# michaelklachko/NoisyNet

Hardware: NVIDIA H100
Metric: NoisyNet CIFAR-10 4-bit training images/sec (higher is better)
Workload: dtype bf16

## Files before the change

### noisynet_b200/csrc/nn_conv_umma.cu

```cuda
#include <cuda_bf16.h>
#include <stdio.h>
#include <stdlib.h>

#include "nn_common.cuh"
#include "nn_wgmma.cuh"
#include "nn_conv_tma.h"

namespace {

constexpr int UM_BLOCK_M = 128;
constexpr int UM_BLOCK_K = 64;
constexpr int UM_THREADS = 384;
constexpr int UM_ACC_CH = 4;
constexpr int UM_A_STAGE = UM_BLOCK_M * 128;
constexpr int UM_MAX_NT = 120;

struct UmmaP {
    int B, H, W, Cp;
    int KH, KW, stride, pad, OH, OW;
    int M, Cout, n_t, n_mma, num_kb, stages, acc_cols;
    int main_col, sig_col, wsum_col;
    int ring_bytes;
    const __nv_bfloat16* xp;
    const __nv_bfloat16* wp;
// ... 328 lines not shown
            s_plain = nn_warp_sum(s_plain); s_abs = nn_warp_sum(s_abs); s_max = nn_warp_max(s_max);
            if (lane == 0) {
                atomicAdd(p.stats + 0, s_plain);
                atomicAdd(p.stats + 1, s_abs);
                nn_atomic_max_float(p.stats + 2, s_max);
            }
        }
    }
    if (dbg && tid == 128) { dbg[4] = clock64(); unsigned smid; asm volatile("mov.u32 %0, %%smid;" : "=r"(smid)); dbg[7] = smid; }
}


struct SplitEpiP {
    const float* partial; int splits, n_tiles, n_mma, n_t, main_col, sig_col, m_pad, M, Cout;
    float y_scale, s_scale, current; const float* scale_dev; nn_rng rng; float *y, *y_noisy; int noisy;
    double* stat_partial; unsigned* stat_counters; BnFinP fin; float* zero_out;
};
__global__ void __launch_bounds__(256)
k_splitk_epilogue(const SplitEpiP p) {
    const int ngrp = (p.Cout + 3) >> 2;
    const int total = p.M * ngrp;
    float coef = 0.f;
    NnRng rs = {0, 0, 0, 0};
    if (p.noisy) { coef = nn_noise_coef(*p.scale_dev, p.current); rs = nn_rng_load(p.rng); }
    for (int i = blockIdx.x * blockDim.x + threadIdx.x; i < total; i += gridDim.x * blockDim.x) {
        const int m = i % p.M, g = i / p.M;
        const int n0 = g * 4;
        const int tile = n0 / p.n_t, c0 = n0 - tile * p.n_t;
        float am[4] = {0.f, 0.f, 0.f, 0.f}, as[4] = {0.f, 0.f, 0.f, 0.f};
        for (int z = 0; z < p.splits; ++z) {
            const float* src = p.partial + (((size_t)z * p.n_tiles + tile) * p.n_mma) * p.m_pad + m;
#pragma unroll
            for (int j = 0; j < 4; ++j) {
                am[j] += src[(size_t)(p.main_col + c0 + j) * p.m_pad];
                if (p.noisy) as[j] += src[(size_t)(p.sig_col + c0 + j) * p.m_pad];
            }
        }
        float zz[4] = {0.f, 0.f, 0.f, 0.f};
        if (p.noisy) nn_normal4(rs, (uint64_t)m * ngrp + (uint64_t)g, zz);
        float* o = (p.noisy ? p.y_noisy : p.y) + (size_t)m * p.Cout + n0;
        float ov[4] = {0.f, 0.f, 0.f, 0.f};
#pragma unroll
        for (int j = 0; j < 4; ++j) {
            if (n0 + j < p.Cout) {
                const float yv = am[j] * p.y_scale;
                ov[j] = p.noisy ? __fadd_rn(yv, __fmul_rn(zz[j], nn_sigma(coef, as[j] * p.s_scale))) : yv;
                o[j] = ov[j];
                if (p.noisy && p.y) p.y[(size_t)m * p.Cout + n0 + j] = yv;
            }
        }
        if (p.stat_partial) {
            __shared__ double sh[8][8];
            const int lane = threadIdx.x & 31, wi = threadIdx.x >> 5;
#pragma unroll
            for (int j = 0; j < 4; ++j) {
                double s1 = (double)ov[j], s2 = (double)ov[j] * (double)ov[j];
#pragma unroll
                for (int o2 = 16; o2 > 0; o2 >>= 1) { s1 += __shfl_xor_sync(0xffffffffu, s1, o2); s2 += __shfl_xor_sync(0xffffffffu, s2, o2); }
                if (lane == 0) { sh[wi][2 * j] = s1; sh[wi][2 * j + 1] = s2; }
            }
            __syncthreads();
            if (threadIdx.x < 4 && n0 + (int)threadIdx.x < p.Cout) {
                const int j = threadIdx.x, c = n0 + j, slices = p.M >> 8, slice = (m >> 8);
                double a1 = 0.0, a2 = 0.0;
#pragma unroll
                for (int w = 0; w < 8; ++w) { a1 += sh[w][2 * j]; a2 += sh[w][2 * j + 1]; }
                double* part = p.stat_partial + (size_t)c * slices * 2;
                part[slice * 2] = a1; part[slice * 2 + 1] = a2;
                __threadfence();
                if (atomicAdd(p.stat_counters + c, 1u) == (unsigned)slices - 1u) {
                    p.stat_counters[c] = 0u;
                    __threadfence();
                    bn_finalize_channel(part, slices, 2, c, p.fin);
                    if (c == 0 && p.zero_out) *p.zero_out = 0.f;
                }
            }
        }
    }
}

constexpr int SH_MAX_PAIRS = 64;
constexpr int SH_STAGES = 2;
constexpr int SH_MAX_N = 256;
constexpr int SH_POOL_IT = 5;

struct ShiftP {
    int H, W, OH, OW, KH, KW, Cout;
    int n_mma, main_col, sig_col, n_pairs;
    int a_pixels, a_stage, b_bytes, n_tiles;
    long long total_pixels;
    const __nv_bfloat16 *xp, *wp;
    float y_scale, s_scale;
    float *y, *y_noisy;
    float* pooled;
    uint8_t* pool_arg;
    int blk, tiles_x, tiles_per_img, sbo_units;
    double* stat_partial;
    unsigned* stat_ticket;
    BnFinP fin;
    float* zero_out;
    const float* z_inject;
    float current;
    const float* scale_dev;
    nn_rng rng;
    int* err_flag;
    long long* dbg;
};

__device__ __forceinline__ long long shift_tile_v0(const ShiftP& p, int t, int& b, int& r0, int& c0) {
    if (!p.blk) { b = 0; r0 = 0; c0 = 0; return (long long)t * UM_BLOCK_M; }
    b = t / p.tiles_per_img;
    const int rem = t - b * p.tiles_per_img, rb = rem / p.tiles_x;
    r0 = rb * 16; c0 = (rem - rb * p.tiles_x) * 8;
    return ((long long)b * p.H + r0) * p.W + c0;
}
__device__ __forceinline__ bool shift_tile_live(const ShiftP& p, int t) {
    if (p.blk) {
        const int rem = t % p.tiles_per_img, rb = rem / p.tiles_x;
        return rb * 16 < p.OH && (rem - rb * p.tiles_x) * 8 < p.OW;
    }
    const unsigned v0 = (unsigned)t * UM_BLOCK_M, total = (unsigned)p.total_pixels;
    unsigned v1 = v0 + UM_BLOCK_M - 1;
    if (v1 >= total) v1 = total - 1;
    const unsigned hw = (unsigned)(p.H * p.W);
    const unsigned b0 = v0 / hw, b1 = v1 / hw;
    if (b0 != b1) return true;
    return (int)((v0 - b0 * hw) / (unsigned)p.W) < p.OH;
}

template <int MODE, int SH_EPI_WARPS, bool POOL>
__global__ void __launch_bounds__((1 + SH_EPI_WARPS) * 32, 1)
k_conv_shift(const ShiftP p) {
    constexpr bool NOISY = MODE != 0;
    constexpr int SH_THREADS = (1 + SH_EPI_WARPS) * 32;
    static_assert(SH_EPI_WARPS >= 8 && SH_EPI_WARPS % 4 == 0, "the first 8 epilogue warps are the MMA warpgroups");
    extern __shared__ uint8_t smem_raw[];
    const uint32_t base = (smem_u32(smem_raw) + 127u) & ~127u;
    const uint32_t b_base = base;
    const uint32_t a_base = b_base + (uint32_t)p.b_bytes;
    const uint32_t bar_base = a_base + (uint32_t)SH_STAGES * (uint32_t)p.a_stage;
    const uint32_t a_full = bar_base, a_empty = bar_base + 8u * SH_STAGES;
    const uint32_t b_full = bar_base + 16u * SH_STAGES;
    const uint32_t abort_slot = b_full + 8u, tab_slot = abort_slot + 4u;
    const uint32_t pool_slot = (tab_slot + 4u * SH_MAX_PAIRS + 15u) & ~15u;
    const uint32_t acc_slot = pool_slot + 12u * 1024u;
    uint8_t* gen0 = smem_raw + (base - smem_u32(smem_raw));
    const AccTile acc_tile = {reinterpret_cast<float*>(gen0 + (acc_slot - base)), p.n_mma + 4};
    volatile uint32_t* abort_g = reinterpret_cast<volatile uint32_t*>(gen0 + (abort_slot - base));
    uint32_t* tap_tab = reinterpret_cast<uint32_t*>(gen0 + (tab_slot - base));

    const int tid = threadIdx.x, lane = tid & 31;
    const int warp = __shfl_sync(0xffffffffu, tid >> 5, 0);
    if (tid < p.n_pairs) {
        const int khw = p.KH * p.KW, t0 = 2 * tid, t1 = 2 * tid + 1;
        const int sh0 = (t0 / p.KW) * p.W + (t0 % p.KW);
        const int sh1 = t1 < khw ? (t1 / p.KW) * p.W + (t1 % p.KW) : sh0 + 1;
        tap_tab[tid] = (uint32_t)sh0 | ((uint32_t)(sh1 - sh0) << 16);
    }
    if (tid == 0) {
        for (int s = 0; s < SH_STAGES; ++s) { mbar_init(a_full + 8 * s, 1); mbar_init(a_empty + 8 * s, 2); }
        mbar_init(b_full, 1);
        *abort_g = 0;
        fence_mbar_init();
    }
    {
        uint4* az = reinterpret_cast<uint4*>(gen0 + (a_base - base));
        const int n16 = SH_STAGES * p.a_stage / 16;
        for (int i = tid; i < n16; i += SH_THREADS) az[i] = make_uint4(0, 0, 0, 0);
        fence_proxy_async();
    }
    __syncthreads();
    const int hw = p.H * p.W;

    if (warp == SH_EPI_WARPS) {
        if (elect_one_sync()) {
            mbar_arrive_expect_tx(b_full, (uint32_t)p.b_bytes);
            bulk_g2s(b_base, p.wp, (uint32_t)p.b_bytes, b_full);
        }
        __syncwarp();
        int s = 0;
        uint32_t ph = 1u;
        for (int t = blockIdx.x; t < p.n_tiles; t += gridDim.x) {
            if (!shift_tile_live(p, t)) continue;
            if (!mbar_wait(a_empty + 8 * s, ph)) { *abort_g = 1; break; }
            if (*abort_g) break;
            int tb, tr0, tc0;
            const long long v0 = shift_tile_v0(p, t, tb, tr0, tc0);
            long long px = p.total_pixels - v0;
            if (px > p.a_pixels) px = p.a_pixels;
            const uint32_t bytes = (uint32_t)px * 16u;
            if (elect_one_sync()) {
                mbar_arrive_expect_tx(a_full + 8 * s, bytes);
                bulk_g2s(a_base + (uint32_t)s * p.a_stage, p.xp + v0 * 8, bytes, a_full + 8 * s);
            }
            __syncwarp();
            if (++s == SH_STAGES) { s = 0; ph ^= 1u; }
        }
    } else {
        const bool mma_wg = warp < 8;
        const int wg = warp >> 2;
        if (mma_wg && !mbar_wait(b_full, 0)) *abort_g = 2;
        int s = 0;
        uint32_t ph = 0u;
        const uint64_t bd0 = gmma_desc_none(b_base, (uint32_t)p.n_mma, 8u);
        const uint64_t ad_t = gmma_desc_none(0u, 0u, (uint32_t)p.sbo_units);
        const int q = warp & 3, jq = warp >> 2;
        constexpr int per_q = SH_EPI_WARPS / 4;
        const int ohw = p.OH * p.OW;
        const int ngrp = (p.Cout + 3) >> 2;
        float coef = 0.f;
        NnRng rs = {0, 0, 0, 0};
        if (NOISY) coef = nn_noise_coef(*p.scale_dev, p.current);
        if (MODE == 1) rs = nn_rng_load(p.rng);
        const float y_scale = p.y_scale, s_scale = p.s_scale;
        float st1[SH_POOL_IT], st2[SH_POOL_IT];
#pragma unroll
        for (int it = 0; it < SH_POOL_IT; ++it) { st1[it] = 0.f; st2[it] = 0.f; }
        int i = 0;
        for (int t = blockIdx.x; t < p.n_tiles; t += gridDim.x) {
            if (!shift_tile_live(p, t)) continue;
            if (mma_wg && !*abort_g) {
                if (!mbar_wait(a_full + 8 * s, ph)) {
                    *abort_g = 4;
                } else {
                    if (p.dbg && i < 32 && warp == 0 && lane == 0) p.dbg[((size_t)blockIdx.x * 32 + i) * 4 + 0] = clock64();
                    const uint32_t a_s = a_base + (uint32_t)s * p.a_stage + (uint32_t)wg * 128u * (uint32_t)p.sbo_units;
                    for (int c = 0; 64 * c < p.n_mma; ++c) {
                        const int n = min(64, p.n_mma - 64 * c);
                        float acc[1][32];
                        wg_fence();
#pragma unroll 1
                        for (int j = 0; j < p.n_pairs; ++j) {
                            const uint32_t e = tap_tab[j];
                            const uint64_t ad = ad_t | (uint64_t)(((a_s >> 4) + (e & 0xFFFFu)) & 0x3FFFu) | ((uint64_t)((e >> 16) & 0x3FFFu) << 16);
                            wgmma_n<0, 0>(acc[0], ad, bd0 + (uint64_t)(2 * j * p.n_mma + 64 * c), n, j != 0);
                        }
                        wg_commit();
                        wg_wait_all();
                        wg_fence_regs<32>(acc[0]);
                        wg_acc_store(acc, acc_tile, 64 * wg, 64 * c, n);
                    }
                    __syncwarp();
                    if ((warp & 3) == 0 && elect_one_sync()) mbar_arrive(a_empty + 8 * s);
                    __syncwarp();
                    if (p.dbg && i < 32 && warp == 0 && lane == 0) p.dbg[((size_t)blockIdx.x * 32 + i) * 4 + 1] = clock64();
                }
                if (++s == SH_STAGES) { s = 0; ph ^= 1u; }
            }
            named_bar_sync(1, SH_EPI_WARPS * 32);
            if (*abort_g) break;
            if (p.dbg && i < 32 && warp == 0 && lane == 0) p.dbg[((size_t)blockIdx.x * 32 + i) * 4 + 2] = clock64();
            int b, ih, iw;
            bool row_ok;
            if (p.blk) {
                int r0, c0;
                shift_tile_v0(p, t, b, r0, c0);
                ih = r0 + q * 4 + (lane >> 3); iw = c0 + (lane & 7);
                row_ok = ih < p.OH && iw < p.OW;
            } else {
                const unsigned v = (unsigned)t * UM_BLOCK_M + q * 32 + lane;
                b = (int)(v / (unsigned)hw);
                const int rem = (int)(v - (unsigned)b * (unsigned)hw);
                ih = (int)((unsigned)rem / (unsigned)p.W); iw = rem - ih * p.W;
                row_ok = v < (unsigned)p.total_pixels && ih < p.OH && iw < p.OW;
            }
            const int pix = ih * p.OW + iw;
            const uint64_t grp_row = (uint64_t)((long long)b * ohw + pix) * ngrp;
            const size_t out_row = (size_t)b * p.Cout * ohw + pix;
            float* const out_main = (NOISY ? p.y_noisy : p.y) + out_row;
            float* const out_y = (NOISY && p.y) ? p.y + out_row : nullptr;
            const uint32_t t_lane = (uint32_t)(q * 32) << 16;
            if (POOL) {
                const int PW = p.OW >> 1, PHW = (p.OH >> 1) * PW;
                const int w = (lane & 1) | ((lane >> 2) & 2);
                const bool w1 = (w & 1) != 0, w2 = (w & 2) != 0;
                const size_t pbase = (size_t)b * p.Cout * PHW + (size_t)(ih >> 1) * PW + (iw >> 1);
                const bool warp_live = __any_sync(0xffffffffu, row_ok);
                const int n_fix = ngrp / per_q, g_extra = n_fix * per_q;
                auto pool_group = [&](const float (&v)[4], int nb, float& s1, float& s2) {
                    const float s01 = w1 ? v[1] : v[0], s10 = w1 ? v[0] : v[1], s23 = w1 ? v[3] : v[2], s32 = w1 ? v[2] : v[3];
                    const float own = w2 ? s23 : s01;
                    const float c1 = w2 ? s32 : s10;
                    const float c2 = w2 ? s01 : s23;
                    const float c3 = w2 ? s10 : s32;
                    const float a1 = __shfl_xor_sync(0xffffffffu, c1, 1), a2 = __shfl_xor_sync(0xffffffffu, c2, 8),
                                a3 = __shfl_xor_sync(0xffffffffu, c3, 9);
                    float m = own; int a = w;
                    if (a1 > m || (a1 == m && (w ^ 1) < a)) { m = a1; a = w ^ 1; }
                    if (a2 > m || (a2 == m && (w ^ 2) < a)) { m = a2; a = w ^ 2; }
                    if (a3 > m || (a3 == m && (w ^ 3) < a)) { m = a3; a = w ^ 3; }
                    if (row_ok && nb + w < p.Cout) {
                        const size_t o = pbase + (size_t)(nb + w) * PHW;
                        p.pooled[o] = m;
                        p.pool_arg[o] = (uint8_t)a;
                        s1 += m; s2 = fmaf(m, m, s2);
                    }
                };
                auto noisy_values = [&](const float (&am)[4], const float (&as)[4], const float (&z)[4], int nb, float (&v)[4]) {
#pragma unroll
                    for (int j = 0; j < 4; ++j) {
                        v[j] = am[j] * y_scale;
                        if (NOISY) {
                            const float zz = MODE == 2 ? ((row_ok && nb + j < p.Cout) ? __ldg(p.z_inject + out_row + (size_t)(nb + j) * ohw) : 0.f) : z[j];
                            v[j] = __fadd_rn(v[j], __fmul_rn(zz, nn_sigma(coef, as[j] * s_scale)));
                        }
                    }
                };
#pragma unroll
                for (int it = 0; it < SH_POOL_IT; ++it) {
                    if (MODE == 1 && (it & 1) == 0 && it + 1 < SH_POOL_IT - 1) {
                        if (it + 1 < n_fix) {
                            if (!warp_live) continue;
                            const int ga = jq + it * per_q, gb = ga + per_q;
                            float am[4], as[4], bm[4], bs[4], za[4], zb[4], va[4], vb[4];
                            acc_ld4x4(acc_tile, t_lane + (uint32_t)(p.main_col + ga * 4), t_lane + (uint32_t)(p.sig_col + ga * 4),
                                       t_lane + (uint32_t)(p.main_col + gb * 4), t_lane + (uint32_t)(p.sig_col + gb * 4), am, as, bm, bs);
                            nn_normal4(rs, grp_row + (uint64_t)ga, za);
                            nn_normal4(rs, grp_row + (uint64_t)gb, zb);
                            noisy_values(am, as, za, ga * 4, va);
                            noisy_values(bm, bs, zb, gb * 4, vb);
                            pool_group(va, ga * 4, st1[it], st2[it]);
                            pool_group(vb, gb * 4, st1[it + 1], st2[it + 1]);
                            continue;
                        }
                    } else if (MODE == 1 && (it & 1) == 1 && it < SH_POOL_IT - 1) {
                        if (it < n_fix) continue;
                    }
                    int g4;
                    if (it < SH_POOL_IT - 1) { g4 = jq + it * per_q; if (it >= n_fix) continue; }
                    else { g4 = g_extra; if (g4 >= ngrp || (i % per_q) != jq) continue; }
                    if (!warp_live) continue;
                    float am[4], as[4];
                    if (NOISY) acc_ld4x2(acc_tile, t_lane + (uint32_t)(p.main_col + g4 * 4), t_lane + (uint32_t)(p.sig_col + g4 * 4), am, as);
                    else acc_ld4(acc_tile, t_lane + (uint32_t)(p.main_col + g4 * 4), am);
                    const int nb = g4 * 4;
                    float z[4] = {0.f, 0.f, 0.f, 0.f};
                    if (MODE == 1) nn_normal4(rs, grp_row + (uint64_t)g4, z);
                    float v[4];
                    noisy_values(am, as, z, nb, v);
                    pool_group(v, nb, st1[it], st2[it]);
                }
            } else
            {
            auto one_group = [&](int g4) {
                float am[4], as[4];
                if (NOISY) acc_ld4x2(acc_tile, t_lane + (uint32_t)(p.main_col + g4 * 4), t_lane + (uint32_t)(p.sig_col + g4 * 4), am, as);
                else acc_ld4(acc_tile, t_lane + (uint32_t)(p.main_col + g4 * 4), am);
                if (!row_ok) return;
                const int nb = g4 * 4;
                float z[4];
                if (MODE == 1) nn_normal4(rs, grp_row + (uint64_t)g4, z);
                float* o = out_main + (size_t)nb * ohw;
                if (nb + 4 <= p.Cout && (!NOISY || out_y == nullptr) && MODE != 2) {
                    float* o_run = o;
                    asm volatile("" : "+l"(o_run));
#pragma unroll
                    for (int j = 0; j < 4; ++j) {
                        const float yv = am[j] * y_scale;
                        st_global_f32(o_run, NOISY ? __fadd_rn(yv, __fmul_rn(z[j], nn_sigma(coef, as[j] * s_scale))) : yv);
                        o_run += ohw;
                    }
                    return;
                }
                const int nvalid = min(4, p.Cout - nb);
                float* oy = out_y ? out_y + (size_t)nb * ohw : nullptr;
#pragma unroll
                for (int j = 0; j < 4; ++j) {
                    if (j < nvalid) {
                        const float yv = am[j] * y_scale;
                        if (NOISY) {
                            const float sg = nn_sigma(coef, as[j] * s_scale);
                            const float zz = MODE == 2 ? __ldg(p.z_inject + out_row + (size_t)(nb + j) * ohw) : z[j];
                            o[(size_t)j * ohw] = __fadd_rn(yv, __fmul_rn(zz, sg));
                            if (oy) oy[(size_t)j * ohw] = yv;
                        } else {
                            o[(size_t)j * ohw] = yv;
                        }
                    }
                }
            };
            const bool hot = MODE == 1 && out_y == nullptr;
            for (int g4 = (jq + i) % per_q; g4 < ngrp; g4 += 2 * per_q) {
                const int g4b = g4 + per_q;
                if (hot && g4b * 4 + 4 <= p.Cout) {
                    float am[4], as[4], bm[4], bs[4];
                    acc_ld4x4(acc_tile, t_lane + (uint32_t)(p.main_col + g4 * 4), t_lane + (uint32_t)(p.sig_col + g4 * 4),
                               t_lane + (uint32_t)(p.main_col + g4b * 4), t_lane + (uint32_t)(p.sig_col + g4b * 4), am, as, bm, bs);
                    if (!row_ok) continue;
                    float za[4], zb[4];
                    nn_normal4(rs, grp_row + (uint64_t)g4, za);
                    nn_normal4(rs, grp_row + (uint64_t)g4b, zb);
                    float* oa = out_main + (size_t)(g4 * 4) * ohw;
                    float* ob = out_main + (size_t)(g4b * 4) * ohw;
                    asm volatile("" : "+l"(oa), "+l"(ob));
#pragma unroll
                    for (int j = 0; j < 4; ++j) {
                        st_global_f32(oa, __fadd_rn(am[j] * y_scale, __fmul_rn(za[j], nn_sigma(coef, as[j] * s_scale))));
                        st_global_f32(ob, __fadd_rn(bm[j] * y_scale, __fmul_rn(zb[j], nn_sigma(coef, bs[j] * s_scale))));
                        oa += ohw; ob += ohw;
                    }
                    continue;
                }
                one_group(g4);
                if (g4b < ngrp) one_group(g4b);
            }
            }
            named_bar_sync(1, SH_EPI_WARPS * 32);
            if (p.dbg && i < 32 && warp == 0 && lane == 0) p.dbg[((size_t)blockIdx.x * 32 + i) * 4 + 3] = clock64();
            ++i;
        }
        if (POOL && p.stat_partial) {
            float* ssum = reinterpret_cast<float*>(gen0 + (pool_slot - base));
            const int w = (lane & 1) | ((lane >> 2) & 2);
#pragma unroll
            for (int it = 0; it < SH_POOL_IT; ++it) {
                float a1 = st1[it], a2 = st2[it];
#pragma unroll
                for (int o = 2; o <= 16; o <<= 1) {
                    if (o == 8) continue;
                    a1 += __shfl_xor_sync(0xffffffffu, a1, o); a2 += __shfl_xor_sync(0xffffffffu, a2, o);
                }
                if ((lane & ~9) == 0) { ssum[((warp * SH_POOL_IT + it) * 4 + w) * 2] = a1; ssum[((warp * SH_POOL_IT + it) * 4 + w) * 2 + 1] = a2; }
            }
            asm volatile("bar.sync 1, %0;" ::"r"(SH_EPI_WARPS * 32) : "memory");
            const int et = tid;
            if (et < p.Cout) {
                const int g4 = et >> 2, j = et & 3, n_fix = ngrp / per_q;
                double d1 = 0.0, d2 = 0.0;
                if (g4 < n_fix * per_q) {
                    const int it = g4 / per_q, wj = g4 - it * per_q;
#pragma unroll
                    for (int k = 0; k < 4; ++k) {
                        d1 += (double)ssum[(((wj * 4 + k) * SH_POOL_IT + it) * 4 + j) * 2];
                        d2 += (double)ssum[(((wj * 4 + k) * SH_POOL_IT + it) * 4 + j) * 2 + 1];
                    }
                } else {
                    for (int k = 0; k < SH_EPI_WARPS; ++k) {
                        d1 += (double)ssum[((k * SH_POOL_IT + SH_POOL_IT - 1) * 4 + j) * 2];
                        d2 += (double)ssum[((k * SH_POOL_IT + SH_POOL_IT - 1) * 4 + j) * 2 + 1];
                    }
                }
                p.stat_partial[((size_t)blockIdx.x * p.Cout + et) * 2] = d1;
                p.stat_partial[((size_t)blockIdx.x * p.Cout + et) * 2 + 1] = d2;
                __threadfence();
            }
            asm volatile("bar.sync 1, %0;" ::"r"(SH_EPI_WARPS * 32) : "memory");
            volatile int* last_g = reinterpret_cast<volatile int*>(ssum);
            if (et == 0) *last_g = (atomicAdd(p.stat_ticket, 1u) == gridDim.x - 1) ? 1 : 0;
            asm volatile("bar.sync 1, %0;" ::"r"(SH_EPI_WARPS * 32) : "memory");
            if (*last_g) {
                __threadfence();
                if (et < p.Cout) bn_finalize_channel(p.stat_partial + (size_t)et * 2, (int)gridDim.x, (int64_t)p.Cout * 2, et, p.fin);
                if (et == 0) { *p.stat_ticket = 0u; if (p.zero_out) *p.zero_out = 0.f; }
            }
        } else if (p.zero_out && blockIdx.x == 0 && tid == 0) {
            *p.zero_out = 0.f;
        }
    }
    __syncthreads();
    if (*abort_g && tid == 0) nn_pipeline_abort(p.err_flag, 200 + (int)*abort_g);
}

__global__ void __launch_bounds__(256)
k_pack_act(const float* __restrict__ x, __nv_bfloat16* __restrict__ xp, int B, int C, int HW, int Cp, float code_scale) {
    const int chunks = Cp >> 3;
    const int64_t total = (int64_t)B * HW * chunks;
    for (int64_t i = blockIdx.x * (int64_t)blockDim.x + threadIdx.x; i < total; i += (int64_t)gridDim.x * blockDim.x) {
        const int64_t pixel = i % ((int64_t)B * HW);
        const int chunk = (int)(i / ((int64_t)B * HW));
        const int b = (int)(pixel / HW), p = (int)(pixel - (int64_t)b * HW);
        __align__(16) __nv_bfloat16 v[8];
#pragma unroll
        for (int j = 0; j < 8; ++j) {
            const int c = chunk * 8 + j;
            float f = 0.f;
            if (c < C) {
                f = __ldg(x + ((int64_t)b * C + c) * HW + p);
                if (code_scale > 0.f) f = rintf(__fdiv_rn(f, code_scale));
            }
            v[j] = __float2bfloat16_rn(f);
        }
        *reinterpret_cast<uint4*>(xp + (pixel * Cp + chunk * 8)) = *reinterpret_cast<const uint4*>(v);
    }
}

struct PackWP {
    const float *w_eff, *w_raw;
    __nv_bfloat16* wp;
    int Cout, Cin, KHW, Cp, n_t, n_mma, num_kb, n_tiles;
    int main_col, sig_col, wsum_col, noise_mode, mode;
    int layout;
// ... 567 lines not shown
#pragma unroll
    for (int e = 0; e < 4; ++e) {
        if (c0 + e >= p.Cin) break;
        float t = v[e] * p.scale;
        const size_t o = ((size_t)n * p.Cin + c0 + e) * p.KHW + tap;
        if (p.w_raw) { const float w = __ldg(p.w_raw + o); if (w > p.hi || w < p.lo) t = 0.f; }
        p.gw[o] = t;
    }
}

struct Plan {
    int Cp, K_total, num_kb, n_tiles, n_t, n_mma, acc_cols, stages, main_col, sig_col, wsum_col, ring_bytes;
    size_t xp_bytes, wp_bytes, smem_bytes;
};

static inline int pad_to(int v, int a) { return (v + a - 1) / a * a; }

static Plan make_plan(int Cin_k, int KHW, int n_out, bool has_main, bool has_sigma, bool has_wsum, int64_t pixels_in,
                      int m_tiles_hint = 0) {
    Plan pl;
    pl.Cp = pad_to(Cin_k, 8);
    pl.K_total = KHW * pl.Cp;
    pl.num_kb = (pl.K_total + UM_BLOCK_K - 1) / UM_BLOCK_K;
    const int env_max_nt = UM_MAX_NT;
    const int max_nt = has_sigma ? (has_main ? env_max_nt : 248) : 256;
    pl.n_tiles = (n_out + max_nt - 1) / max_nt;
    if (m_tiles_hint > 0) {
        while (m_tiles_hint * pl.n_tiles < 96 && (n_out + pl.n_tiles - 1) / pl.n_tiles > 48) pl.n_tiles *= 2;
    }
    pl.n_t = pad_to((n_out + pl.n_tiles - 1) / pl.n_tiles, 8);
    pl.n_tiles = (n_out + pl.n_t - 1) / pl.n_t;
    int col = 0;
    pl.main_col = pl.sig_col = pl.wsum_col = -1;
    if (has_main) { pl.main_col = col; col += pl.n_t; }
    if (has_sigma) { pl.sig_col = col; col += pl.n_t; }
    if (has_wsum) { pl.wsum_col = col; col += 1; }
    pl.n_mma = pad_to(col, 16);
    if (pl.n_mma < 16) pl.n_mma = 16;
    int need = pl.n_mma;
    if (has_main) need = max(need, pl.main_col + pad_to(pl.n_t, 16));
    if (has_sigma) need = max(need, pl.sig_col + pad_to(pl.n_t, 16));
    if (has_wsum) need = max(need, pl.wsum_col + 16);
    pl.acc_cols = need;
    const int stage_bytes = UM_A_STAGE + pl.n_mma * 128;
    const int max_stages = 4;
    pl.stages = (192 * 1024) / stage_bytes;
    if (pl.stages > max_stages) pl.stages = max_stages;
    if (pl.stages < 2) pl.stages = 2;
    if (pl.stages > pl.num_kb) pl.stages = pl.num_kb < 1 ? 1 : pl.num_kb;
    const int acc_bytes = UM_BLOCK_M * (pl.acc_cols + 4) * 4;
    pl.ring_bytes = pad_to(max(pl.stages * stage_bytes, acc_bytes), 1024);
    pl.smem_bytes = 1024 + (size_t)pl.ring_bytes + 16 * pl.stages + 64;
    pl.xp_bytes = (size_t)pixels_in * pl.Cp * 2;
    pl.wp_bytes = (size_t)pl.n_tiles * pl.num_kb * pl.n_mma * 64 * 2;
    return pl;
}

static inline size_t align_up(size_t v, size_t a) { return (v + a - 1) / a * a; }

struct ShiftPlan {
    int n_t, n_mma, main_col, sig_col, n_chunks, n_pairs, a_pixels, a_stage, b_bytes, n_tiles;
    size_t smem_bytes, wp_bytes;
};
int g_shift_enable = 1;

static bool make_shift_plan(const nn_conv_geom& g, bool noisy, ShiftPlan* out) {
    if (!g_shift_enable) return false;
    if (g.Cin > 8 || g.stride != 1 || g.pad != 0 || g.KH > g.H || g.KW > g.W || g.W >= 4096) return false;
    if ((int64_t)g.B * g.H * g.W >= (int64_t)1 << 31) return false;
    ShiftPlan sp;
    sp.n_t = pad_to(g.Cout, 8);
    sp.main_col = 0;
    sp.sig_col = noisy ? sp.n_t : -1;
    sp.n_mma = pad_to(noisy ? 2 * sp.n_t : sp.n_t, 16);
    if (sp.n_mma > SH_MAX_N) return false;
    const int khw = g.KH * g.KW;
    sp.n_pairs = (khw + 1) / 2;
    sp.n_chunks = 2 * sp.n_pairs;
    sp.a_pixels = UM_BLOCK_M + (g.KH - 1) * g.W + (g.KW - 1) + 8;
    sp.a_stage = pad_to(sp.a_pixels * 16, 128);
    sp.b_bytes = sp.n_chunks * sp.n_mma * 16;
    sp.n_tiles = (int)(((int64_t)g.B * g.H * g.W + UM_BLOCK_M - 1) / UM_BLOCK_M);
    const int a_stage_blk = pad_to(((15 + g.KH - 1) * g.W + 8 + (g.KW - 1) + 8) * 16, 128);
    sp.smem_bytes = 128 + (size_t)sp.b_bytes + (size_t)SH_STAGES * (a_stage_blk > sp.a_stage ? a_stage_blk : sp.a_stage) + 16 * SH_STAGES + 64 +
                    4 * SH_MAX_PAIRS + 16 + 12 * 1024 + (size_t)UM_BLOCK_M * (sp.n_mma + 4) * 4;
    if (sp.n_pairs > SH_MAX_PAIRS) return false;
    sp.wp_bytes = (size_t)sp.b_bytes;
    if (sp.smem_bytes > 227 * 1024) return false;
    if (out) *out = sp;
    return true;
}

long long* g_dbg_buf = nullptr;
size_t g_dbg_ctas = 0, g_dbg_last = 0;

int g_time_main = 0;
cudaEvent_t g_ev0 = nullptr, g_ev1 = nullptr;

static int nn_num_sms_cached() {
    int dev = 0;
    cudaGetDevice(&dev);
    return nn_num_sms(dev);
}

static int launch_umma(const UmmaP& p, const Plan& pl, cudaStream_t st, void* splitk_ws = nullptr, size_t splitk_ws_bytes = 0) {
    NN_ONCE_PER_DEVICE({
        NN_CUDA_OK(cudaFuncSetAttribute(k_conv_umma<0>, cudaFuncAttributeMaxDynamicSharedMemorySize, 227 * 1024));
        NN_CUDA_OK(cudaFuncSetAttribute(k_conv_umma<1>, cudaFuncAttributeMaxDynamicSharedMemorySize, 227 * 1024));
        NN_CUDA_OK(cudaFuncSetAttribute(k_conv_umma<2>, cudaFuncAttributeMaxDynamicSharedMemorySize, 227 * 1024));
    });
    const bool extras = p.bias || p.mask_x || p.z_inject || p.z_export || p.sigma_export || p.stats;
    int epi = 0;
    if (!extras && p.main_col >= 0 && p.noise_mode != NN_NOISE_NONE && p.y_noisy) epi = 1;
    else if (!extras && p.main_col >= 0 && p.noise_mode == NN_NOISE_NONE && p.y) epi = 2;
    UmmaP pd = p;
    pd.inc_taps = epi == 2 ? 1 : 0;
    pd.rows_tile = UM_BLOCK_M;
    dim3 grid((p.M + pd.rows_tile - 1) / pd.rows_tile, pl.n_tiles);
#ifdef NN_KDEBUG
    static const bool want_dbg = getenv("NN_UMMA_DEBUG") != nullptr;
    if (want_dbg) {
        const size_t ctas = (size_t)grid.x * grid.y;
        if (ctas > g_dbg_ctas) {
            if (g_dbg_buf) cudaFree(g_dbg_buf);
            cudaMalloc(&g_dbg_buf, ctas * 8 * sizeof(long long));
            g_dbg_ctas = ctas;
        }
        cudaMemsetAsync(g_dbg_buf, 0, ctas * 8 * sizeof(long long), st);
        pd.dbg = g_dbg_buf;
        g_dbg_last = ctas;
    }
#else
    const bool want_dbg = false;
#endif
    int splits = 1;
    if ((epi == 1 || epi == 2) && p.OH * p.OW == 1 && !want_dbg && (int)(grid.x * grid.y) * 2 <= nn_num_sms_cached() && pl.num_kb >= 8 && splitk_ws) {
        splits = 4;
        while (splits > 1 && pl.num_kb / splits < 4) --splits;
        const size_t need = (size_t)splits * pl.n_tiles * pl.n_mma * grid.x * UM_BLOCK_M * sizeof(float);
        if (need > splitk_ws_bytes) splits = 1;
    }
    if (splits > 1) {
        grid.z = splits;
        pd.partial = (float*)splitk_ws;
        pd.m_pad = (int)grid.x * UM_BLOCK_M;
    }
#ifdef NN_KDEBUG
    static const bool want_kdbg = getenv("NN_UMMA_KDEBUG") != nullptr;
    if (want_kdbg) {
        const size_t rows = ((size_t)grid.x * grid.y * pl.num_kb * 4 + 7) / 8;
        if (rows > g_dbg_ctas) {
            if (g_dbg_buf) cudaFree(g_dbg_buf);
            cudaMalloc(&g_dbg_buf, rows * 8 * sizeof(long long));
            g_dbg_ctas = rows;
        }
        cudaMemsetAsync(g_dbg_buf, 0, rows * 8 * sizeof(long long), st);
        pd.kdbg = g_dbg_buf;
        g_dbg_last = rows;
    }
#endif
    if (g_time_main) {
        if (!g_ev0) { cudaEventCreate(&g_ev0); cudaEventCreate(&g_ev1); }
        cudaEventRecord(g_ev0, st);
    }
    UmmaAMap amap;
    memset(&amap, 0, sizeof(amap));
    if (nn_debug_tma_enable(-1) && p.OH * p.OW == 1 && p.pad == 0 && p.KH == p.H && p.KW == p.W && pd.rows_tile == UM_BLOCK_M &&
// ... 99 lines not shown
    if (cudaMemcpy(&v, f, sizeof(int), cudaMemcpyDeviceToHost) != cudaSuccess) return -3;
    if (reset) cudaMemset(f, 0, sizeof(int));
    return v;
}

extern "C" int nn_conv_pool_fusable(const nn_conv_geom* g, int32_t noise_mode, int32_t precision);

static int shift_conv_fwd(const nn_conv_fwd_args* a, const ShiftPlan& sp, int device, cudaStream_t st) {
    const nn_conv_geom& g = a->g;
    int OH, OW;
    nn_out_hw(g, OH, OW);
    const bool noise = a->noise_mode != NN_NOISE_NONE;
    const size_t xp_bytes = (size_t)g.B * g.H * g.W * 16;
    uint8_t* ws = (uint8_t*)align_up((size_t)a->workspace, 1024);
    const size_t need = (a->x_packed ? 0 : align_up(xp_bytes, 1024)) + (a->w_packed ? 0 : align_up(sp.wp_bytes, 1024)) + 1024;
    if ((!a->x_packed || !a->w_packed) && (!a->workspace || (size_t)a->workspace_bytes < need))
        return nn_fail("nn_noisy_conv_fwd: workspace too small%s (need %lld bytes)", "", (long long)need);
    const __nv_bfloat16* xp = (const __nv_bfloat16*)a->x_packed;
    const __nv_bfloat16* wp = (const __nv_bfloat16*)a->w_packed;
    if (!xp) {
        const int64_t total = (int64_t)g.B * g.H * g.W;
        int grid = (int)((total + 255) / 256);
        if (grid > 16 * nn_num_sms(device)) grid = 16 * nn_num_sms(device);
        k_pack_act<<<grid, 256, 0, st>>>(a->x, (__nv_bfloat16*)ws, g.B, g.Cin, g.H * g.W, 8, a->a_code_scale);
        NN_LAUNCH_OK();
        xp = (const __nv_bfloat16*)ws;
        ws += align_up(xp_bytes, 1024);
    }
    if (!wp) {
        PackWP pw;
        memset(&pw, 0, sizeof(pw));
        pw.w_eff = a->w_eff; pw.w_raw = a->w_raw; pw.wp = (__nv_bfloat16*)ws;
        pw.Cout = g.Cout; pw.Cin = g.Cin; pw.KHW = g.KH * g.KW; pw.Cp = 8; pw.n_t = sp.n_t; pw.n_mma = sp.n_mma;
        pw.num_kb = sp.n_chunks; pw.n_tiles = 1; pw.main_col = sp.main_col; pw.sig_col = sp.sig_col; pw.wsum_col = -1;
        pw.noise_mode = a->noise_mode; pw.mode = 0; pw.layout = NN_PACK_SHIFT; pw.w_code_scale = a->w_code_scale;
        const int64_t total = (int64_t)sp.n_chunks * sp.n_mma;
        k_pack_w<<<(int)((total + 255) / 256), 256, 0, st>>>(pw);
        NN_LAUNCH_OK();
        wp = (const __nv_bfloat16*)ws;
    }
    ShiftP p;
    memset(&p, 0, sizeof(p));
    p.H = g.H; p.W = g.W; p.OH = OH; p.OW = OW; p.KH = g.KH; p.KW = g.KW; p.Cout = g.Cout;
    p.n_mma = sp.n_mma; p.main_col = sp.main_col; p.sig_col = sp.sig_col; p.n_pairs = sp.n_pairs;
    p.a_pixels = sp.a_pixels; p.a_stage = sp.a_stage; p.b_bytes = sp.b_bytes; p.n_tiles = sp.n_tiles;
    p.total_pixels = (long long)g.B * g.H * g.W;
    p.xp = xp; p.wp = wp;
    const float as = a->a_code_scale > 0.f ? a->a_code_scale : 1.f;
    const float wsc = a->w_code_scale > 0.f ? a->w_code_scale : 1.f;
    p.y_scale = as * wsc; p.s_scale = as;
    p.y = a->y; p.y_noisy = a->y_noisy; p.z_inject = a->z_inject;
    p.pooled = a->pooled_out; p.pool_arg = a->argmax_out;
    p.current = a->current; p.scale_dev = a->scale_dev; p.rng = a->rng;
    p.err_flag = nn_umma_err_flag(device);
    p.sbo_units = 8; p.zero_out = a->zero_out;
    if (p.pooled) {
        p.blk = 1; p.tiles_x = g.W / 8; p.tiles_per_img = (g.H / 16) * p.tiles_x; p.sbo_units = g.W;
        p.n_tiles = g.B * p.tiles_per_img;
        p.a_pixels = (15 + g.KH - 1) * g.W + 8 + (g.KW - 1) + 8;
        p.a_stage = pad_to(p.a_pixels * 16, 128);
        if (a->bn_mean) {
            if (!a->bn_invstd || !a->bn_scratch) return nn_fail("nn_noisy_conv_fwd: bn_mean needs bn_invstd and bn_scratch%s", "");
            if (a->bn_eval_mode && (!a->bn_running_mean || !a->bn_running_var))
                return nn_fail("nn_noisy_conv_fwd: bn_eval_mode needs the running statistics%s", "");
            p.stat_ticket = (unsigned*)a->bn_scratch;
            p.stat_partial = (double*)((uint8_t*)a->bn_scratch + 16);
            p.fin.count = (double)g.B * (OH / 2) * (OW / 2);
            p.fin.eps = a->bn_eps; p.fin.momentum = a->bn_momentum; p.fin.mean = a->bn_mean; p.fin.invstd = a->bn_invstd;
            p.fin.running_mean = a->bn_running_mean; p.fin.running_var = a->bn_running_var; p.fin.xmax_out = nullptr;
            p.fin.eval_mode = a->bn_eval_mode;
        }
    } else if (a->bn_mean) {
        return nn_fail("nn_noisy_conv_fwd: bn_mean is served together with pooled_out only%s", "");
    }
    int grid = nn_num_sms(device);
    if (grid > p.n_tiles) grid = p.n_tiles;
    if (p.stat_partial && grid > 256) grid = 256;
#ifdef NN_KDEBUG
    static const bool want_dbg = getenv("NN_UMMA_DEBUG") != nullptr;
#else
    const bool want_dbg = false;
#endif
    if (want_dbg) {
        const size_t rows = (size_t)grid * 16;
        if (rows > g_dbg_ctas) {
            if (g_dbg_buf) cudaFree(g_dbg_buf);
            cudaMalloc(&g_dbg_buf, rows * 8 * sizeof(long long));
            g_dbg_ctas = rows;
        }
        cudaMemsetAsync(g_dbg_buf, 0, rows * 8 * sizeof(long long), st);
        p.dbg = g_dbg_buf;
        g_dbg_last = rows;
    }
    if (g_time_main) {
        if (!g_ev0) { cudaEventCreate(&g_ev0); cudaEventCreate(&g_ev1); }
        cudaEventRecord(g_ev0, st);
    }
    const int mode = !noise ? 0 : (a->z_inject ? 2 : 1);
#define NN_SHIFT_LAUNCH(MODE, EW, POOL)                                                                                \
    do {                                                                                                               \
        NN_ONCE_PER_DEVICE({ \
            NN_CUDA_OK(cudaFuncSetAttribute(k_conv_shift<MODE, EW, POOL>, cudaFuncAttributeMaxDynamicSharedMemorySize, 227 * 1024)); \
        });                                                                                                              \
        k_conv_shift<MODE, EW, POOL><<<grid, (1 + EW) * 32, sp.smem_bytes, st>>>(p);                                    \
    } while (0)
    if (p.pooled) {
        if (mode == 0) NN_SHIFT_LAUNCH(0, 16, true); else if (mode == 1) NN_SHIFT_LAUNCH(1, 16, true); else NN_SHIFT_LAUNCH(2, 16, true);
    } else {
        if (mode == 0) NN_SHIFT_LAUNCH(0, 16, false); else if (mode == 1) NN_SHIFT_LAUNCH(1, 16, false); else NN_SHIFT_LAUNCH(2, 16, false);
    }
#undef NN_SHIFT_LAUNCH
    if (g_time_main) cudaEventRecord(g_ev1, st);
    NN_LAUNCH_OK();
    return 0;
}

extern "C" int nn_conv_pack_layout(const nn_conv_geom* g, int32_t noise_mode, int32_t precision) {
    if (!g || precision != NN_PREC_BF16) return NN_PACK_TILED;
    if (make_shift_plan(*g, noise_mode != NN_NOISE_NONE, nullptr)) return NN_PACK_SHIFT;
    int OH, OW;
    nn_out_hw(*g, OH, OW);
    return nn_tma_make_plan(g->Cin, g->KH, g->KW, g->stride, g->pad, g->Cout, noise_mode != NN_NOISE_NONE, OH, OW, nullptr) ? NN_PACK_TMA
                                                                                                                          : NN_PACK_TILED;
}
extern "C" int nn_conv_dgrad_pack_layout(const nn_conv_geom* g, int32_t precision) {
    if (!g || precision != NN_PREC_BF16 || g->stride != 1) return NN_PACK_TILED;
    return nn_tma_make_plan(g->Cout, g->KH, g->KW, 1, g->KH - 1 - g->pad, g->Cin, false, g->H, g->W, nullptr) ? NN_PACK_TMA : NN_PACK_TILED;
}
extern "C" int nn_conv_pool_fusable(const nn_conv_geom* g, int32_t noise_mode, int32_t precision) {
    if (!g || precision != NN_PREC_BF16) return 0;
    if (!make_shift_plan(*g, noise_mode != NN_NOISE_NONE, nullptr)) return 0;
    int OH, OW;
    nn_out_hw(*g, OH, OW);
    const int ngrp = (g->Cout + 3) / 4;
    return g->W % 8 == 0 && g->H % 16 == 0 && OH % 2 == 0 && OW % 2 == 0 && ngrp / 4 <= SH_POOL_IT - 1 && ngrp % 4 <= 1;
}
extern "C" int nn_conv_linear_bn_fusable(const nn_conv_geom* g, int32_t noise_mode, int32_t precision, int device) {
    if (!g || precision != NN_PREC_BF16) return 0;
    int OH, OW;
    nn_out_hw(*g, OH, OW);
    const int M = g->B * OH * OW;
    if (OH * OW != 1 || M % 256 || M > 4096) return 0;
    const Plan pl = make_plan(g->Cin, g->KH * g->KW, g->Cout, true, noise_mode != NN_NOISE_NONE, false, (int64_t)g->B * g->H * g->W, (M + 127) / 128);
    const int ctas = ((M + UM_BLOCK_M - 1) / UM_BLOCK_M) * pl.n_tiles;
    return ctas * 2 <= nn_num_sms(device) && pl.num_kb >= 8 && pl.num_kb / 2 >= 4;
}
extern "C" int64_t nn_conv_bn_scratch_bytes(int Cout) { return 16 + (int64_t)256 * Cout * 2 * sizeof(double); }
extern "C" int nn_debug_shift_enable(int enable) {
    const int prev = g_shift_enable;
    if (enable >= 0) g_shift_enable = enable;
    return prev;
}

static void fill_pack_tma(PackWP& pw, const TmaPlan& tp) {
    pw.Cp = tp.Cp; pw.n_t = tp.n_t; pw.n_mma = tp.n_mma; pw.num_kb = 0; pw.n_tiles = tp.n_tiles;
    pw.main_col = tp.main_col; pw.sig_col = tp.sig_col; pw.wsum_col = -1; pw.layout = NN_PACK_TMA;
    pw.t_nc64 = tp.n_c64; pw.t_tail = tp.tail_w; pw.t_nc = tp.nc; pw.t_wt = tp.wt; pw.t_nhalf = tp.n_half; pw.t_tapbytes = tp.tap_bytes;
}
static int64_t pack_tma_chunks(const TmaPlan& tp) { return (int64_t)tp.n_tiles * tp.n_mma * tp.taps * (tp.wt >> 3); }

static bool tma_fwd_plan(const nn_conv_fwd_args* a, TmaPlan* tp) {
    const nn_conv_geom& g = a->g;
    int OH, OW;
    nn_out_hw(g, OH, OW);
    const bool noise = a->noise_mode != NN_NOISE_NONE;
    const bool has_main = a->w_eff != nullptr || a->w_packed != nullptr;
    const bool lean = has_main && !a->bias && !a->z_export && !a->sigma_export && !a->stats && !a->pooled_out && !a->bn_mean && !(noise && a->y);
    return lean && nn_tma_make_plan(g.Cin, g.KH, g.KW, g.stride, g.pad, g.Cout, noise, OH, OW, tp);
}

static int tma_conv_fwd(const nn_conv_fwd_args* a, const TmaPlan& tp, int device, cudaStream_t st) {
    const nn_conv_geom& g = a->g;
    int OH, OW;
    nn_out_hw(g, OH, OW);
    const size_t xp_bytes = (size_t)g.B * g.H * g.W * tp.Cp * 2;
    const size_t need = (a->x_packed ? 0 : align_up(xp_bytes, 1024)) + (a->w_packed ? 0 : align_up(tp.wp_bytes, 1024)) + 1024;
    if ((!a->x_packed || !a->w_packed) && (!a->workspace || (size_t)a->workspace_bytes < need))
        return nn_fail("nn_noisy_conv_fwd: workspace too small%s (need %lld bytes)", "", (long long)need);
    uint8_t* ws = (uint8_t*)align_up((size_t)a->workspace, 1024);
    const void* xp = a->x_packed;
    const void* wp = a->w_packed;
    if (!xp) {
        const int64_t total = (int64_t)g.B * g.H * g.W * (tp.Cp / 8);
        int grid = (int)((total + 255) / 256);
        if (grid > 16 * nn_num_sms(device)) grid = 16 * nn_num_sms(device);
        k_pack_act<<<grid, 256, 0, st>>>(a->x, (__nv_bfloat16*)ws, g.B, g.Cin, g.H * g.W, tp.Cp, a->a_code_scale);
        NN_LAUNCH_OK();
// ... 639 lines not shown
```

Baseline: 447,200.

## Warp-specialize shift conv: dedicated MMA warpgroups overlapped with epilogue via mbarriers

Splits the shift-conv kernel into two dedicated MMA warpgroups, each owning half of the 128-row tile, and 16 separate epilogue warps. Per-half acc_full/acc_empty mbarriers replace the block-wide named barriers, so the MMA of the next tile can overlap the epilogue of the current one. The MMA loop is templated on N with fixed 4-deep wgmma chains instead of a runtime-N loop, and the TMA loader moves into the first MMA warp. This raises the thread count to 768 and adds more barrier handshakes, but the epilogue no longer stalls the tensor cores between tiles.

```diff
diff --git a/noisynet_b200/csrc/nn_conv_umma.cu b/noisynet_b200/csrc/nn_conv_umma.cu
--- a/noisynet_b200/csrc/nn_conv_umma.cu
+++ b/noisynet_b200/csrc/nn_conv_umma.cu
@@ -434,6 +434,7 @@
 constexpr int SH_MAX_PAIRS = 64;
 constexpr int SH_STAGES = 2;
 constexpr int SH_MAX_N = 256;
+constexpr int SH_MAX_N1 = 80;
 constexpr int SH_POOL_IT = 5;
 
 struct ShiftP {
@@ -459,6 +460,11 @@
     long long* dbg;
 };
 
+constexpr int SH_DBG = 8;
+__device__ __forceinline__ void shift_dbg(const ShiftP& p, int i, int k) {
+    if (p.dbg && i < 32) p.dbg[((size_t)blockIdx.x * 32 + i) * SH_DBG + k] = clock64();
+}
+
 __device__ __forceinline__ long long shift_tile_v0(const ShiftP& p, int t, int& b, int& r0, int& c0) {
     if (!p.blk) { b = 0; r0 = 0; c0 = 0; return (long long)t * UM_BLOCK_M; }
     b = t / p.tiles_per_img;
@@ -480,12 +486,131 @@
     return (int)((v0 - b0 * hw) / (unsigned)p.W) < p.OH;
 }
 
+template <int N, int L>
+__device__ __forceinline__ void shift_chain(float* acc, const uint32_t* tap_tab, uint64_t ad_t, uint32_t a16, uint64_t bd, uint32_t b_pair,
+                                            int j0) {
+    wg_fence();
+#pragma unroll
+    for (int k = 0; k < L; ++k) {
+        const uint32_t e = tap_tab[j0 + k];
+        const uint64_t ad = ad_t | (uint64_t)((a16 + (e & 0xFFFFu)) & 0x3FFFu) | ((uint64_t)((e >> 16) & 0x3FFFu) << 16);
+        wgmma_c<N, 0, 0>(acc, ad, bd + (uint64_t)(j0 + k) * b_pair, j0 + k != 0);
+    }
+    wg_commit();
+}
+template <int N>
+__device__ __forceinline__ void shift_half_mma(float* acc, const uint32_t* tap_tab, uint64_t ad_t, uint32_t a16, uint64_t bd, uint32_t b_pair,
+                                               int n_pairs) {
+    for (int j0 = 0; j0 < n_pairs; j0 += 4) {
+        switch (min(4, n_pairs - j0)) {
+            case 4: shift_chain<N, 4>(acc, tap_tab, ad_t, a16, bd, b_pair, j0); break;
+            case 3: shift_chain<N, 3>(acc, tap_tab, ad_t, a16, bd, b_pair, j0); break;
+            case 2: shift_chain<N, 2>(acc, tap_tab, ad_t, a16, bd, b_pair, j0); break;
+            default: shift_chain<N, 1>(acc, tap_tab, ad_t, a16, bd, b_pair, j0); break;
+        }
+    }
+    wg_wait_all();
+    wg_fence_regs<N / 2>(acc);
+}
+template <int N>
+__device__ __forceinline__ void shift_acc_store(const float* acc, const AccTile& t, int row0, int col0) {
+    const int wt = threadIdx.x & 127, l = wt & 31;
+    float* r0 = t.p + (size_t)(row0 + 16 * (wt >> 5) + (l >> 2)) * t.stride + col0 + 2 * (l & 3);
+    float* r1 = r0 + 8 * t.stride;
+#pragma unroll
+    for (int i = 0; i < N / 8; ++i) {
+        *reinterpret_cast<float2*>(r0 + 8 * i) = make_float2(acc[4 * i], acc[4 * i + 1]);
+        *reinterpret_cast<float2*>(r1 + 8 * i) = make_float2(acc[4 * i + 2], acc[4 * i + 3]);
+    }
+}
+
+__host__ __device__ constexpr int shift_passes(int nc) {
+    int np = 1;
+    while (nc / np > SH_MAX_N1 || nc % (8 * np) != 0) ++np;
+    return np;
+}
+
+__device__ __forceinline__ void shift_load_next(const ShiftP& p, uint32_t a_base, uint32_t a_full, int s, bool loader, int& t_ld) {
+    while (t_ld < p.n_tiles && !shift_tile_live(p, t_ld)) t_ld += gridDim.x;
+    if (t_ld >= p.n_tiles) return;
+    if (loader) {
+        int tb, tr0, tc0;
+        const long long v0 = shift_tile_v0(p, t_ld, tb, tr0, tc0);
+        long long px = p.total_pixels - v0;
+        if (px > p.a_pixels) px = p.a_pixels;
+        const uint32_t bytes = (uint32_t)px * 16u;
+        if (elect_one_sync()) {
+            mbar_arrive_expect_tx(a_full + 8 * s, bytes);
+            bulk_g2s(a_base + (uint32_t)s * p.a_stage, p.xp + v0 * 8, bytes, a_full + 8 * s);
+        }
+        __syncwarp();
+    }
+    t_ld += gridDim.x;
+}
+
+template <int NC>
+__device__ __forceinline__ uint32_t shift_mma_role(const ShiftP& p, int h, uint32_t a_base, uint32_t b_base, uint32_t a_full,
+                                                   uint32_t a_empty, uint32_t b_full, uint32_t acc_full, uint32_t acc_empty,
+                                                   const uint32_t* tap_tab, const AccTile& acc_tile, volatile uint32_t* abort_g) {
+    static_assert(SH_STAGES == 2, "k_conv_shift: stage and phase are derived from the tile count");
+    constexpr int NP = shift_passes(NC), N = NC / NP;
+    const bool first_warp = (threadIdx.x & 127) < 32, loader = h == 0 && first_warp;
+    if (loader) {
+        if (elect_one_sync()) {
+            mbar_arrive_expect_tx(b_full, (uint32_t)p.b_bytes);
+            bulk_g2s(b_base, p.wp, (uint32_t)p.b_bytes, b_full);
+        }
+        __syncwarp();
+    }
+    int t_ld = blockIdx.x;
+    if (loader) {
+        shift_load_next(p, a_base, a_full, 0, true, t_ld);
+        shift_load_next(p, a_base, a_full, 1, true, t_ld);
+    }
+    if (!mbar_wait(b_full, 0)) return 2;
+    const uint64_t bd0 = gmma_desc_none(b_base, (uint32_t)NC, 8u);
+    const uint64_t ad_t = gmma_desc_none(0u, 0u, (uint32_t)p.sbo_units);
+    const uint32_t b_pair = 2u * NC;
+    int i = 0;
+    for (int t = blockIdx.x; t < p.n_tiles; t += gridDim.x) {
+        if (!shift_tile_live(p, t)) continue;
+        const int s = i & 1;
+        const uint32_t ph = ((uint32_t)i >> 1) & 1u;
+        if (!mbar_wait(a_full + 8 * s, ph)) return 4;
+        if (*abort_g) return 0;
+        if (loader && (threadIdx.x & 31) == 0) shift_dbg(p, i, 0);
+        const uint32_t a16h = ((a_base + (uint32_t)s * p.a_stage) >> 4) + (uint32_t)h * 8u * (uint32_t)p.sbo_units;
+#pragma unroll
+        for (int c = 0; c < NP; ++c) {
+            float acc[N / 2];
+            shift_half_mma<N>(acc, tap_tab, ad_t, a16h, bd0 + (uint64_t)(c * N), b_pair, p.n_pairs);
+            if (c == NP - 1) {
+                if (h == 1) {
+                    if (first_warp && elect_one_sync()) mbar_arrive(a_empty + 8 * s);
+                    __syncwarp();
+                } else if (loader) {
+                    if (!mbar_wait(a_empty + 8 * s, ph)) return 8;
+                    shift_load_next(p, a_base, a_full, s, true, t_ld);
+                }
+            }
+            if (c == 0 && !mbar_wait(acc_empty + 8 * h, ((uint32_t)i & 1u) ^ 1u)) return 6;
+            shift_acc_store<N>(acc, acc_tile, 64 * h, c * N);
+        }
+        __syncwarp();
+        if (elect_one_sync()) mbar_arrive(acc_full + 8 * h);
+        __syncwarp();
+        if (first_warp && (threadIdx.x & 31) == 0) shift_dbg(p, i, 1 + h);
+        ++i;
+    }
+    return 0;
+}
+
 template <int MODE, int SH_EPI_WARPS, bool POOL>
-__global__ void __launch_bounds__((1 + SH_EPI_WARPS) * 32, 1)
+__global__ void __launch_bounds__((SH_EPI_WARPS + 8) * 32, 1)
 k_conv_shift(const ShiftP p) {
     constexpr bool NOISY = MODE != 0;
-    constexpr int SH_THREADS = (1 + SH_EPI_WARPS) * 32;
-    static_assert(SH_EPI_WARPS >= 8 && SH_EPI_WARPS % 4 == 0, "the first 8 epilogue warps are the MMA warpgroups");
+    constexpr int SH_THREADS = (SH_EPI_WARPS + 8) * 32;
+    static_assert(SH_EPI_WARPS >= 8 && SH_EPI_WARPS % 4 == 0, "the MMA warpgroups start on a warpgroup boundary");
     extern __shared__ uint8_t smem_raw[];
     const uint32_t base = (smem_u32(smem_raw) + 127u) & ~127u;
     const uint32_t b_base = base;
@@ -493,7 +618,8 @@
     const uint32_t bar_base = a_base + (uint32_t)SH_STAGES * (uint32_t)p.a_stage;
     const uint32_t a_full = bar_base, a_empty = bar_base + 8u * SH_STAGES;
     const uint32_t b_full = bar_base + 16u * SH_STAGES;
-    const uint32_t abort_slot = b_full + 8u, tab_slot = abort_slot + 4u;
+    const uint32_t acc_full = b_full + 8u, acc_empty = acc_full + 16u;
+    const uint32_t abort_slot = acc_empty + 16u, tab_slot = abort_slot + 4u;
     const uint32_t pool_slot = (tab_slot + 4u * SH_MAX_PAIRS + 15u) & ~15u;
     const uint32_t acc_slot = pool_slot + 12u * 1024u;
     uint8_t* gen0 = smem_raw + (base - smem_u32(smem_raw));
@@ -510,8 +636,12 @@
         tap_tab[tid] = (uint32_t)sh0 | ((uint32_t)(sh1 - sh0) << 16);
     }
     if (tid == 0) {
-        for (int s = 0; s < SH_STAGES; ++s) { mbar_init(a_full + 8 * s, 1); mbar_init(a_empty + 8 * s, 2); }
+        for (int s = 0; s < SH_STAGES; ++s) { mbar_init(a_full + 8 * s, 1); mbar_init(a_empty + 8 * s, 1); }
         mbar_init(b_full, 1);
+        for (int h = 0; h < 2; ++h) {
+            mbar_init(acc_full + 8 * h, 4);
+            mbar_init(acc_empty + 8 * h, SH_EPI_WARPS / 2);
+        }
         *abort_g = 0;
         fence_mbar_init();
     }
@@ -524,39 +654,23 @@
     __syncthreads();
     const int hw = p.H * p.W;
 
-    if (warp == SH_EPI_WARPS) {
-        if (elect_one_sync()) {
-            mbar_arrive_expect_tx(b_full, (uint32_t)p.b_bytes);
-            bulk_g2s(b_base, p.wp, (uint32_t)p.b_bytes, b_full);
-        }
-        __syncwarp();
-        int s = 0;
-        uint32_t ph = 1u;
-        for (int t = blockIdx.x; t < p.n_tiles; t += gridDim.x) {
-            if (!shift_tile_live(p, t)) continue;
-            if (!mbar_wait(a_empty + 8 * s, ph)) { *abort_g = 1; break; }
-            if (*abort_g) break;
-            int tb, tr0, tc0;
-            const long long v0 = shift_tile_v0(p, t, tb, tr0, tc0);
-            long long px = p.total_pixels - v0;
-            if (px > p.a_pixels) px = p.a_pixels;
-            const uint32_t bytes = (uint32_t)px * 16u;
-            if (elect_one_sync()) {
-                mbar_arrive_expect_tx(a_full + 8 * s, bytes);
-                bulk_g2s(a_base + (uint32_t)s * p.a_stage, p.xp + v0 * 8, bytes, a_full + 8 * s);
-            }
-            __syncwarp();
-            if (++s == SH_STAGES) { s = 0; ph ^= 1u; }
-        }
+    if (warp >= SH_EPI_WARPS) {
+        const int h = (warp - SH_EPI_WARPS) >> 2;
+        uint32_t fail = 0;
+#define NN_SHIFT_MMA(NC)                                                                                                         \
+    case NC:                                                                                                                     \
+        fail = shift_mma_role<NC>(p, h, a_base, b_base, a_full, a_empty, b_full, acc_full, acc_empty, tap_tab, acc_tile, abort_g); \
+        break
+        switch (p.n_mma) {
+            NN_SHIFT_MMA(16); NN_SHIFT_MMA(32); NN_SHIFT_MMA(48); NN_SHIFT_MMA(64); NN_SHIFT_MMA(80); NN_SHIFT_MMA(96);
+            NN_SHIFT_MMA(112); NN_SHIFT_MMA(128); NN_SHIFT_MMA(144); NN_SHIFT_MMA(160); NN_SHIFT_MMA(176); NN_SHIFT_MMA(192);
+            NN_SHIFT_MMA(208); NN_SHIFT_MMA(224); NN_SHIFT_MMA(240); NN_SHIFT_MMA(256);
+            default: fail = 7; break;
+        }
+#undef NN_SHIFT_MMA
+        if (fail) *abort_g = fail;
     } else {
-        const bool mma_wg = warp < 8;
-        const int wg = warp >> 2;
-        if (mma_wg && !mbar_wait(b_full, 0)) *abort_g = 2;
-        int s = 0;
-        uint32_t ph = 0u;
-        const uint64_t bd0 = gmma_desc_none(b_base, (uint32_t)p.n_mma, 8u);
-        const uint64_t ad_t = gmma_desc_none(0u, 0u, (uint32_t)p.sbo_units);
-        const int q = warp & 3, jq = warp >> 2;
+        const int q = warp & 3, jq = warp >> 2, h = q >> 1;
         constexpr int per_q = SH_EPI_WARPS / 4;
         const int ohw = p.OH * p.OW;
         const int ngrp = (p.Cout + 3) >> 2;
@@ -568,40 +682,13 @@
         float st1[SH_POOL_IT], st2[SH_POOL_IT];
 #pragma unroll
         for (int it = 0; it < SH_POOL_IT; ++it) { st1[it] = 0.f; st2[it] = 0.f; }
+        const bool stamp = lane == 0 && (warp == 0 || warp == 2);
         int i = 0;
         for (int t = blockIdx.x; t < p.n_tiles; t += gridDim.x) {
             if (!shift_tile_live(p, t)) continue;
-            if (mma_wg && !*abort_g) {
-                if (!mbar_wait(a_full + 8 * s, ph)) {
-                    *abort_g = 4;
-                } else {
-                    if (p.dbg && i < 32 && warp == 0 && lane == 0) p.dbg[((size_t)blockIdx.x * 32 + i) * 4 + 0] = clock64();
-                    const uint32_t a_s = a_base + (uint32_t)s * p.a_stage + (uint32_t)wg * 128u * (uint32_t)p.sbo_units;
-                    for (int c = 0; 64 * c < p.n_mma; ++c) {
-                        const int n = min(64, p.n_mma - 64 * c);
-                        float acc[1][32];
-                        wg_fence();
-#pragma unroll 1
-                        for (int j = 0; j < p.n_pairs; ++j) {
-                            const uint32_t e = tap_tab[j];
-                            const uint64_t ad = ad_t | (uint64_t)(((a_s >> 4) + (e & 0xFFFFu)) & 0x3FFFu) | ((uint64_t)((e >> 16) & 0x3FFFu) << 16);
-                            wgmma_n<0, 0>(acc[0], ad, bd0 + (uint64_t)(2 * j * p.n_mma + 64 * c), n, j != 0);
-                        }
-                        wg_commit();
-                        wg_wait_all();
-                        wg_fence_regs<32>(acc[0]);
-                        wg_acc_store(acc, acc_tile, 64 * wg, 64 * c, n);
-                    }
-                    __syncwarp();
-                    if ((warp & 3) == 0 && elect_one_sync()) mbar_arrive(a_empty + 8 * s);
-                    __syncwarp();
-                    if (p.dbg && i < 32 && warp == 0 && lane == 0) p.dbg[((size_t)blockIdx.x * 32 + i) * 4 + 1] = clock64();
-                }
-                if (++s == SH_STAGES) { s = 0; ph ^= 1u; }
-            }
-            named_bar_sync(1, SH_EPI_WARPS * 32);
+            if (!mbar_wait(acc_full + 8 * h, (uint32_t)i & 1u)) { *abort_g = 5; break; }
             if (*abort_g) break;
-            if (p.dbg && i < 32 && warp == 0 && lane == 0) p.dbg[((size_t)blockIdx.x * 32 + i) * 4 + 2] = clock64();
+            if (stamp) shift_dbg(p, i, 3 + 2 * h);
             int b, ih, iw;
             bool row_ok;
             if (p.blk) {
@@ -757,8 +844,10 @@
                 if (g4b < ngrp) one_group(g4b);
             }
             }
-            named_bar_sync(1, SH_EPI_WARPS * 32);
-            if (p.dbg && i < 32 && warp == 0 && lane == 0) p.dbg[((size_t)blockIdx.x * 32 + i) * 4 + 3] = clock64();
+            __syncwarp();
+            if (elect_one_sync()) mbar_arrive(acc_empty + 8 * h);
+            __syncwarp();
+            if (stamp) shift_dbg(p, i, 4 + 2 * h);
             ++i;
         }
         if (POOL && p.stat_partial) {
@@ -1492,7 +1581,7 @@
     sp.b_bytes = sp.n_chunks * sp.n_mma * 16;
     sp.n_tiles = (int)(((int64_t)g.B * g.H * g.W + UM_BLOCK_M - 1) / UM_BLOCK_M);
     const int a_stage_blk = pad_to(((15 + g.KH - 1) * g.W + 8 + (g.KW - 1) + 8) * 16, 128);
-    sp.smem_bytes = 128 + (size_t)sp.b_bytes + (size_t)SH_STAGES * (a_stage_blk > sp.a_stage ? a_stage_blk : sp.a_stage) + 16 * SH_STAGES + 64 +
+    sp.smem_bytes = 128 + (size_t)sp.b_bytes + (size_t)SH_STAGES * (a_stage_blk > sp.a_stage ? a_stage_blk : sp.a_stage) + 16 * SH_STAGES + 96 +
                     4 * SH_MAX_PAIRS + 16 + 12 * 1024 + (size_t)UM_BLOCK_M * (sp.n_mma + 4) * 4;
     if (sp.n_pairs > SH_MAX_PAIRS) return false;
     sp.wp_bytes = (size_t)sp.b_bytes;
@@ -1758,7 +1847,7 @@
     const bool want_dbg = false;
 #endif
     if (want_dbg) {
-        const size_t rows = (size_t)grid * 16;
+        const size_t rows = (size_t)grid * 32 * SH_DBG / 8;
         if (rows > g_dbg_ctas) {
             if (g_dbg_buf) cudaFree(g_dbg_buf);
             cudaMalloc(&g_dbg_buf, rows * 8 * sizeof(long long));
@@ -1778,7 +1867,7 @@
         NN_ONCE_PER_DEVICE({ \
             NN_CUDA_OK(cudaFuncSetAttribute(k_conv_shift<MODE, EW, POOL>, cudaFuncAttributeMaxDynamicSharedMemorySize, 227 * 1024)); \
         });                                                                                                              \
-        k_conv_shift<MODE, EW, POOL><<<grid, (1 + EW) * 32, sp.smem_bytes, st>>>(p);                                    \
+        k_conv_shift<MODE, EW, POOL><<<grid, (EW + 8) * 32, sp.smem_bytes, st>>>(p);                                    \
     } while (0)
     if (p.pooled) {
         if (mode == 0) NN_SHIFT_LAUNCH(0, 16, true); else if (mode == 1) NN_SHIFT_LAUNCH(1, 16, true); else NN_SHIFT_LAUNCH(2, 16, true);
```

Result: faster. 471,900 (median of 6 runs) (+5.5%).
